# liuQuan98/APR

Measured on AMD Instinct MI355X. Metric: point-cloud pairs/sec (120k-pt KITTI frame, FCGF encode+match+SVD), higher is better.
Workload: dtype f32

## Files before the change

apr_amd/csrc/ransac.hip:

```cpp
#include <atomic>
#include <cstring>
#include <map>
#include <mutex>
#include <utility>

#include "common.h"
#include "irls.h"
#include "ransac_raw.h"

namespace {

__host__ __device__ inline uint64_t splitmix64(uint64_t z) {
  z = (z ^ (z >> 30)) * 0xBF58476D1CE4E5B9ull;
  z = (z ^ (z >> 27)) * 0x94D049BB133111EBull;
  return z ^ (z >> 31);
}

__host__ __device__ inline uint32_t sample_index(uint64_t seed, uint64_t it, int slot, uint32_t n) {
  uint64_t z = splitmix64(seed + (it * 4ull + (uint64_t)slot + 1ull) * 0x9E3779B97F4A7C15ull);
  return (uint32_t)(((z >> 32) * (uint64_t)n) >> 32);
}

__device__ inline void kabsch4(const double s[4][3], const double t[4][3], double T[12]) {
  double ms[3] = {0, 0, 0}, mt[3] = {0, 0, 0};
#pragma unroll
  for (int i = 0; i < 4; ++i)
#pragma unroll
    for (int d = 0; d < 3; ++d) {
      ms[d] += s[i][d];
      mt[d] += t[i][d];
    }
#pragma unroll
  for (int d = 0; d < 3; ++d) {
    ms[d] *= 0.25;
    mt[d] *= 0.25;
  }
  double S[3][3] = {{0, 0, 0}, {0, 0, 0}, {0, 0, 0}};
#pragma unroll
  for (int i = 0; i < 4; ++i)
#pragma unroll
    for (int a = 0; a < 3; ++a)
#pragma unroll
      for (int b = 0; b < 3; ++b) S[a][b] += (s[i][a] - ms[a]) * (t[i][b] - mt[b]);
  double A[4][4];
  A[0][0] = S[0][0] + S[1][1] + S[2][2];
  A[0][1] = S[1][2] - S[2][1];
  A[0][2] = S[2][0] - S[0][2];
  A[0][3] = S[0][1] - S[1][0];
  A[1][1] = S[0][0] - S[1][1] - S[2][2];
  A[1][2] = S[0][1] + S[1][0];
  A[1][3] = S[2][0] + S[0][2];
  A[2][2] = -S[0][0] + S[1][1] - S[2][2];
  A[2][3] = S[1][2] + S[2][1];
  A[3][3] = -S[0][0] - S[1][1] + S[2][2];
  A[1][0] = A[0][1]; A[2][0] = A[0][2]; A[3][0] = A[0][3];
  A[2][1] = A[1][2]; A[3][1] = A[1][3]; A[3][2] = A[2][3];
  double V[4][4] = {{1, 0, 0, 0}, {0, 1, 0, 0}, {0, 0, 1, 0}, {0, 0, 0, 1}};
  for (int sweep = 0; sweep < 12; ++sweep) {
    double off = 0.0;
#pragma unroll
    for (int p = 0; p < 4; ++p)
#pragma unroll
      for (int q2 = p + 1; q2 < 4; ++q2) off += A[p][q2] * A[p][q2];
    double diag = A[0][0] * A[0][0] + A[1][1] * A[1][1] + A[2][2] * A[2][2] + A[3][3] * A[3][3];
    if (off <= 1e-32 * diag || off == 0.0) break;
#pragma unroll
    for (int p = 0; p < 4; ++p)
#pragma unroll
      for (int q2 = p + 1; q2 < 4; ++q2) {
        double apq = A[p][q2];
        if (apq != 0.0) {
          double theta = (A[q2][q2] - A[p][p]) / (2.0 * apq);
          double tt = (theta >= 0.0 ? 1.0 : -1.0) / (fabs(theta) + sqrt(theta * theta + 1.0));
          double c = 1.0 / sqrt(tt * tt + 1.0), sn = tt * c;
#pragma unroll
          for (int k = 0; k < 4; ++k) {
            double akp = A[k][p], akq = A[k][q2];
            A[k][p] = c * akp - sn * akq;
            A[k][q2] = sn * akp + c * akq;
          }
#pragma unroll
          for (int k = 0; k < 4; ++k) {
            double apk = A[p][k], aqk = A[q2][k];
            A[p][k] = c * apk - sn * aqk;
            A[q2][k] = sn * apk + c * aqk;
          }
#pragma unroll
          for (int k = 0; k < 4; ++k) {
            double vkp = V[k][p], vkq = V[k][q2];
            V[k][p] = c * vkp - sn * vkq;
            V[k][q2] = sn * vkp + c * vkq;
          }
        }
      }
  }
  double best = A[0][0];
  double qw = V[0][0], qx = V[1][0], qy = V[2][0], qz = V[3][0];
#pragma unroll
  for (int j = 1; j < 4; ++j)
    if (A[j][j] > best) {
      best = A[j][j];
      qw = V[0][j]; qx = V[1][j]; qy = V[2][j]; qz = V[3][j];
    }
  double nq = 1.0 / sqrt(qw * qw + qx * qx + qy * qy + qz * qz);
  qw *= nq; qx *= nq; qy *= nq; qz *= nq;
  double R[3][3];
  R[0][0] = 1 - 2 * (qy * qy + qz * qz); R[0][1] = 2 * (qx * qy - qw * qz); R[0][2] = 2 * (qx * qz + qw * qy);
  R[1][0] = 2 * (qx * qy + qw * qz); R[1][1] = 1 - 2 * (qx * qx + qz * qz); R[1][2] = 2 * (qy * qz - qw * qx);
  R[2][0] = 2 * (qx * qz - qw * qy); R[2][1] = 2 * (qy * qz + qw * qx); R[2][2] = 1 - 2 * (qx * qx + qy * qy);
#pragma unroll
  for (int a = 0; a < 3; ++a) {
    T[a * 4 + 0] = R[a][0]; T[a * 4 + 1] = R[a][1]; T[a * 4 + 2] = R[a][2];
    T[a * 4 + 3] = mt[a] - (R[a][0] * ms[0] + R[a][1] * ms[1] + R[a][2] * ms[2]);
  }
}

constexpr int kMini = 32;
__host__ __device__ inline int64_t rec2_rows(int64_t n0) { return ((n0 + 1) / 2 + kMini - 1) / kMini * kMini; }

__global__ void k_pack_pairs(const float* __restrict__ xyz0, const float* __restrict__ xyz1, int64_t n1,
                             const long long* __restrict__ corr, int64_t n0, float4* __restrict__ rec,
                             float* __restrict__ rec2, unsigned* __restrict__ maxn2, float* __restrict__ rec2_live,
                             long long* __restrict__ corr_out) {
  int64_t i = (int64_t)blockIdx.x * blockDim.x + threadIdx.x;
  float sx = 0.f, sy = 0.f, sz = 0.f, tx = 3e18f, ty = 3e18f, tz = 3e18f, m = 0.f;
  if (i < n0) {
    long long j = corr[i];
    if (corr_out) {
      j &= 0xFFFFFFFFll;
      corr_out[i] = j;
    }
    if (j < 0 || j >= n1) j = 0;
    sx = xyz0[3 * i]; sy = xyz0[3 * i + 1]; sz = xyz0[3 * i + 2];
    tx = xyz1[3 * j]; ty = xyz1[3 * j + 1]; tz = xyz1[3 * j + 2];
    rec[2 * i] = make_float4(sx, sy, sz, 0.f);
    rec[2 * i + 1] = make_float4(tx, ty, tz, 0.f);
    m = fmaxf(sx * sx + sy * sy + sz * sz, tx * tx + ty * ty + tz * tz);
  }
  if (i < 2 * rec2_rows(n0)) {
    float* row = rec2 + (i >> 1) * 12 + (i & 1);
    row[0] = sx; row[2] = sy; row[4] = sz; row[6] = tx; row[8] = ty; row[10] = tz;
    float* lrow = rec2_live + (i >> 1) * 12 + (i & 1);
    lrow[0] = 0.f; lrow[2] = 0.f; lrow[4] = 0.f; lrow[6] = 3e18f; lrow[8] = 3e18f; lrow[10] = 3e18f;
  }
  for (int d = 32; d >= 1; d >>= 1) m = fmaxf(m, __shfl_xor(m, d));
  if ((threadIdx.x & 63) == 0 && m > 0.f) atomicMax(maxn2, __float_as_uint(m));
}

__device__ inline void load_samples(const float4* __restrict__ rec, uint64_t seed, long long it, uint32_t n0,
                                    double s[4][3], double t[4][3]) {
#pragma unroll
  for (int j = 0; j < 4; ++j) {
    const uint32_t i = sample_index(seed, (uint64_t)it, j, n0);
    const float4 a = rec[2 * (int64_t)i], b = rec[2 * (int64_t)i + 1];
    s[j][0] = (double)a.x; s[j][1] = (double)a.y; s[j][2] = (double)a.z;
    t[j][0] = (double)b.x; t[j][1] = (double)b.y; t[j][2] = (double)b.z;
  }
}

__device__ inline bool edge_reject(double a2, double b2, double r, double r2) {
  const double rb = b2 * r2;
  if (a2 < rb * (1.0 - 1e-12)) return true;
  if (a2 > rb * (1.0 + 1e-12)) return false;
  return sqrt(a2) < sqrt(b2) * r;
}

constexpr int kCandLists = 64;

__device__ inline bool sample_passes(const float4* __restrict__ rec, uint32_t n0, double edge_ratio, long long it,
                                     uint64_t seed) {
  float4 sf[4], tf[4];
  const double r2 = edge_ratio * edge_ratio;
  const float r2f = (float)r2;
  auto fetch = [&](int j) {
    const uint32_t i = sample_index(seed, (uint64_t)it, j, n0);
    sf[j] = rec[2 * (int64_t)i];
    tf[j] = rec[2 * (int64_t)i + 1];
  };
  auto edge_ok = [&](int a, int b) {
    const float dsx = sf[a].x - sf[b].x, dsy = sf[a].y - sf[b].y, dsz = sf[a].z - sf[b].z;
    const float dtx = tf[a].x - tf[b].x, dty = tf[a].y - tf[b].y, dtz = tf[a].z - tf[b].z;
    const float A = dsx * dsx + dsy * dsy + dsz * dsz, B = dtx * dtx + dty * dty + dtz * dtz;
    constexpr float lo = 1.f - 4e-6f, hi = 1.f + 4e-6f;
    const bool sound = (A == 0.f || A >= 1e-30f) && (B == 0.f || B >= 1e-30f) && A < 3e37f && B < 3e37f;
    if (sound && (A < r2f * B * lo || B < r2f * A * lo)) return false;
    if (sound && A > r2f * B * hi && B > r2f * A * hi) return true;
    const double ds2 = ((double)sf[a].x - (double)sf[b].x) * ((double)sf[a].x - (double)sf[b].x) +
                       ((double)sf[a].y - (double)sf[b].y) * ((double)sf[a].y - (double)sf[b].y) +
                       ((double)sf[a].z - (double)sf[b].z) * ((double)sf[a].z - (double)sf[b].z);
    const double dt2 = ((double)tf[a].x - (double)tf[b].x) * ((double)tf[a].x - (double)tf[b].x) +
                       ((double)tf[a].y - (double)tf[b].y) * ((double)tf[a].y - (double)tf[b].y) +
                       ((double)tf[a].z - (double)tf[b].z) * ((double)tf[a].z - (double)tf[b].z);
    return !(edge_reject(ds2, dt2, edge_ratio, r2) || edge_reject(dt2, ds2, edge_ratio, r2));
  };
  fetch(0);
  fetch(1);
  if (!edge_ok(0, 1)) return false;
  fetch(2);
  if (!(edge_ok(0, 2) && edge_ok(1, 2))) return false;
  fetch(3);
  return edge_ok(0, 3) && edge_ok(1, 3) && edge_ok(2, 3);
}

__device__ inline void append_candidate(bool ok, long long it, long long* __restrict__ cand, int* __restrict__ n_cand,
                                        int sub_cap) {
  const unsigned long long m = __ballot(ok);
  if (m) {
    const int lane = threadIdx.x & 63;
    const int list = blockIdx.x & (kCandLists - 1);
    int base = 0;
    if (lane == __ffsll((long long)m) - 1) base = atomicAdd(n_cand + list, __popcll(m));
    base = __shfl(base, __ffsll((long long)m) - 1);
    if (ok) cand[(int64_t)list * sub_cap + base + __popcll(m & ((1ull << lane) - 1ull))] = it;
  }
}

__global__ __launch_bounds__(256) void k_sample_check(const float4* __restrict__ rec, uint32_t n0, double edge_ratio,
                                                      long long it0, long long it1, uint64_t seed,
                                                      long long* __restrict__ cand, int* __restrict__ n_cand,
                                                      int sub_cap) {
  const long long it = it0 + (long long)blockIdx.x * blockDim.x + threadIdx.x;
  const bool ok = it < it1 && sample_passes(rec, n0, edge_ratio, it, seed);
  append_candidate(ok, it, cand, n_cand, sub_cap);
}

constexpr int kScreenThreads = 1024;
constexpr int kScreenPer = 2;
constexpr int kScreenRound = kScreenThreads * kScreenPer;
constexpr int kScreenQueue = 2 * kScreenRound;
constexpr int kScreenBits = 10;
constexpr int64_t kScreenMaxN0 = (160 * 1024 - kScreenQueue * 4 - 512) / 8;

__global__ void k_pack_small(const float4* __restrict__ rec, int64_t n0, const unsigned* __restrict__ maxn2,
                             unsigned long long* __restrict__ rec8) {
  const int64_t i = (int64_t)blockIdx.x * blockDim.x + threadIdx.x;
  if (i >= ((n0 + 31) & ~(int64_t)31)) return;
  if (i >= n0) {
    rec8[i] = 0ull;
    return;
  }
  const float R = sqrtf(__uint_as_float(*maxn2)) * 1.000001f;
  const float inv_h = R > 0.f ? (float)((1 << kScreenBits) - 1) / (2.f * R) : 0.f;
  auto q = [&](float c) {
    int u = (int)floorf((c + R) * inv_h);
    u = u < 0 ? 0 : (u > (1 << kScreenBits) - 1 ? (1 << kScreenBits) - 1 : u);
    return (unsigned)u;
  };
  const float4 a = rec[2 * i], b = rec[2 * i + 1];
  const unsigned lo = q(a.x) | (q(a.y) << kScreenBits) | (q(a.z) << (2 * kScreenBits));
  const unsigned hi = q(b.x) | (q(b.y) << kScreenBits) | (q(b.z) << (2 * kScreenBits));
  rec8[i] = (unsigned long long)lo | ((unsigned long long)hi << 32);
}

__device__ inline float cell_dist(unsigned a, unsigned b) {
  constexpr unsigned M = (1u << kScreenBits) - 1u;
  const int dx = (int)(a & M) - (int)(b & M), dy = (int)((a >> kScreenBits) & M) - (int)((b >> kScreenBits) & M),
            dz = (int)((a >> (2 * kScreenBits)) & M) - (int)((b >> (2 * kScreenBits)) & M);
  return __builtin_sqrtf((float)(dx * dx + dy * dy + dz * dz));
}

__device__ inline uint32_t sample_index_from(uint64_t z, uint32_t n) {
  z = (z ^ (z >> 30)) * 0xBF58476D1CE4E5B9ull;
  z = (z ^ (z >> 27)) * 0x94D049BB133111EBull;
  z ^= z >> 31;
  return (uint32_t)(((z >> 32) * (uint64_t)n) >> 32);
}

__global__ __launch_bounds__(kScreenThreads) void k_sample_screen(const float4* __restrict__ rec,
                                                                  const unsigned long long* __restrict__ rec8, uint32_t n0,
                                                                  double edge_ratio, long long it0, long long it1,
                                                                  long long per_wg, uint64_t seed,
                                                                  long long* __restrict__ cand, int* __restrict__ n_cand,
                                                                  int sub_cap) {
  extern __shared__ unsigned long long s_rec[];
  const uint32_t n0p = (n0 + 31u) & ~31u;
  unsigned* const s_q = reinterpret_cast<unsigned*>(s_rec + n0p);
  int& s_nq = *reinterpret_cast<int*>(s_q + kScreenQueue);
  const int tid = threadIdx.x, lane = tid & 63;
  {
    typedef unsigned long long u64x2 __attribute__((ext_vector_type(2)));
    const u64x2* src = reinterpret_cast<const u64x2*>(rec8);
    u64x2* dst = reinterpret_cast<u64x2*>(s_rec);
    const uint32_t nv = n0p >> 1;
    for (uint32_t i0 = tid; i0 < nv; i0 += 8 * kScreenThreads) {
      u64x2 t[8];
#pragma unroll
      for (int u = 0; u < 8; ++u)
        if (i0 + u * kScreenThreads < nv) t[u] = src[i0 + u * kScreenThreads];
#pragma unroll
      for (int u = 0; u < 8; ++u)
        if (i0 + u * kScreenThreads < nv) dst[i0 + u * kScreenThreads] = t[u];
    }
  }
  if (tid == 0) s_nq = 0;
  const long long base = it0 + (long long)blockIdx.x * per_wg;
  const long long end = (base + per_wg < it1) ? base + per_wg : it1;
  const float r = (float)edge_ratio, E = 1.75f;
  constexpr uint64_t G = 0x9E3779B97F4A7C15ull;
  auto drain = [&]() {
    const int nq = s_nq;
    for (int c0 = 0; c0 < nq; c0 += kScreenThreads) {
      const int c = c0 + tid;
      const long long it = c < nq ? base + (long long)s_q[c] : 0;
      const bool ok = c < nq && sample_passes(rec, n0, edge_ratio, it, seed);
      append_candidate(ok, it, cand, n_cand, sub_cap);
    }
  };
  __syncthreads();
  uint64_t z0 = seed + (uint64_t)(4 * (base + tid) + 1) * G;
  for (long long rb = base; rb < end; rb += kScreenRound) {
#pragma unroll
    for (int u = 0; u < kScreenPer; ++u) {
      const long long it = rb + u * kScreenThreads + tid;
      bool pass = false;
      if (it < end) {
        const unsigned long long a = s_rec[sample_index_from(z0, n0)];
        const unsigned long long b = s_rec[sample_index_from(z0 + G, n0)];
        const float Ds = cell_dist((unsigned)a, (unsigned)b), Dt = cell_dist((unsigned)(a >> 32), (unsigned)(b >> 32));
        pass = !(Ds + E < r * (Dt - E)) && !(Dt + E < r * (Ds - E));
      }
      z0 += (uint64_t)(4 * kScreenThreads) * G;
      const unsigned long long m = __ballot(pass);
      if (m) {
        int qb = 0;
        if (lane == __ffsll((long long)m) - 1) qb = atomicAdd(&s_nq, __popcll(m));
        qb = __shfl(qb, __ffsll((long long)m) - 1);
        if (pass) s_q[qb + __popcll(m & ((1ull << lane) - 1ull))] = (unsigned)(it - base);
      }
    }
    __syncthreads();
    const int nq_now = s_nq;
    __syncthreads();
    if (nq_now > kScreenQueue - kScreenRound) {
      drain();
      __syncthreads();
      if (tid == 0) s_nq = 0;
      __syncthreads();
    }
  }
  drain();
}

__global__ __launch_bounds__(256) void k_fit_check(const float4* __restrict__ rec, uint32_t n0, double thr_gt,
                                                   uint64_t seed, const long long* __restrict__ cand,
                                                   const int* __restrict__ n_cand, int sub_cap,
                                                   Hyp* __restrict__ hyps, int* __restrict__ n_valid, int cap) {
  __shared__ int s_off[kCandLists + 1];
  if (threadIdx.x < 64) {
    const int c = n_cand[threadIdx.x];
    const int incl = apr_wave_incl_scan(c);
    s_off[threadIdx.x + 1] = incl;
    if (threadIdx.x == 0) s_off[0] = 0;
  }
  __syncthreads();
  const int nc = s_off[kCandLists];
  for (int c = blockIdx.x * blockDim.x + threadIdx.x; c < nc; c += gridDim.x * blockDim.x) {
    int list = 0;
#pragma unroll
    for (int step = kCandLists / 2; step >= 1; step >>= 1)
      if (s_off[list + step] <= c) list += step;
    const long long it = cand[(int64_t)list * sub_cap + (c - s_off[list])];
    double s[4][3], t[4][3];
    load_samples(rec, seed, it, n0, s, t);
    double T[12];
    kabsch4(s, t, T);
    bool ok = true;
#pragma unroll
    for (int j = 0; j < 4; ++j) {
      double dx = T[0] * s[j][0] + T[1] * s[j][1] + T[2] * s[j][2] + T[3] - t[j][0];
      double dy = T[4] * s[j][0] + T[5] * s[j][1] + T[6] * s[j][2] + T[7] - t[j][1];
      double dz = T[8] * s[j][0] + T[9] * s[j][1] + T[10] * s[j][2] + T[11] - t[j][2];
      if (dx * dx + dy * dy + dz * dz > thr_gt) ok = false;
    }
    if (!ok) continue;
    const int slot = atomicAdd(n_valid, 1);
    if (slot < cap) {
#pragma unroll
      for (int k = 0; k < 12; ++k) hyps[slot].T[k] = T[k];
      hyps[slot].it = it;
      hyps[slot].inliers = 0;
      hyps[slot].err2 = 0.0;
    }
  }
}

constexpr int kGeoGrid = 2048;
struct GeoPart {
  double e2;
  int cnt;
  int pad;
};

__device__ inline int geo_parts(int nv, int64_t n0) {
  const int nchunk = (int)((n0 + 255) >> 8);
  int S = nv > 0 ? kGeoGrid / nv : 1;
  if (S > nchunk) S = nchunk;
  return S < 1 ? 1 : S;
}

constexpr int kScoreThreads = 256;
__device__ inline int score_parts(int nv, int64_t n0) {
  const int nblk = (int)((n0 + 4 * kScoreThreads - 1) / (4 * kScoreThreads));
  int S = nv > 0 ? kGeoGrid / nv : 1;
  if (S > nblk) S = nblk;
  return S < 1 ? 1 : S;
}

__global__ __launch_bounds__(kScoreThreads) void k_score(const float4* __restrict__ rec, int64_t n0, double thr_lt,
                                               Hyp* __restrict__ hyps, const int* __restrict__ sel_hdr,
                                               const int* __restrict__ sel, GeoPart* __restrict__ part) {
  constexpr int NW = kScoreThreads / 64;
  __shared__ int s_cnt[NW];
  __shared__ double s_e2[NW];
  const int lane = threadIdx.x & 63, wave = threadIdx.x >> 6;
  const int nv = sel_hdr[0];
  const int S = score_parts(nv, n0);
  const int64_t nblk = (n0 + 4 * kScoreThreads - 1) / (4 * kScoreThreads);
  for (int64_t item = blockIdx.x; item < (int64_t)nv * S; item += gridDim.x) {
    const int hs = (int)(item / S), pp = (int)(item - (int64_t)hs * S);
    const int h = sel[hs];
    const int64_t i_begin = (nblk * pp / S) * (4 * kScoreThreads);
    const int64_t i_end = min((long long)((nblk * (pp + 1) / S) * (4 * kScoreThreads)), (long long)n0);
    double T[12];
#pragma unroll
    for (int k = 0; k < 12; ++k) T[k] = hyps[h].T[k];
    int cnt = 0;
    double e2 = 0.0;
    for (int64_t i0 = i_begin + threadIdx.x; i0 < i_end; i0 += 4 * kScoreThreads) {
      float4 a[4], b[4];
#pragma unroll
      for (int u = 0; u < 4; ++u) {
        const int64_t i = i0 + u * kScoreThreads;
        if (i < i_end) {
          a[u] = rec[2 * i];
          b[u] = rec[2 * i + 1];
        }
      }
#pragma unroll
      for (int u = 0; u < 4; ++u) {
        if (i0 + u * kScoreThreads >= i_end) break;
        const double sx = a[u].x, sy = a[u].y, sz = a[u].z;
        double dx = T[0] * sx + T[1] * sy + T[2] * sz + T[3] - (double)b[u].x;
        double dy = T[4] * sx + T[5] * sy + T[6] * sz + T[7] - (double)b[u].y;
        double dz = T[8] * sx + T[9] * sy + T[10] * sz + T[11] - (double)b[u].z;
        double d2 = dx * dx + dy * dy + dz * dz;
        if (d2 < thr_lt) {
          ++cnt;
          e2 += d2;
        }
      }
    }
    for (int d = 32; d >= 1; d >>= 1) {
      cnt += __shfl_xor(cnt, d);
      e2 += __shfl_xor(e2, d);
    }
    if (lane == 0) {
      s_cnt[wave] = cnt;
      s_e2[wave] = e2;
    }
    __syncthreads();
    if (threadIdx.x == 0) {
      int c = 0;
      double e = 0.0;
      for (int w = 0; w < NW; ++w) {
        c += s_cnt[w];
        e += s_e2[w];
      }
      if (S == 1) {
        hyps[h].inliers = c;
        hyps[h].err2 = e;
      } else {
        part[item].cnt = c;
        part[item].e2 = e;
      }
    }
    __syncthreads();
  }
}

__global__ void k_score_finish(Hyp* __restrict__ hyps, const int* __restrict__ sel_hdr, const int* __restrict__ sel,
                               int64_t n0, const GeoPart* __restrict__ part) {
  const int nv = sel_hdr[0];
  const int S = score_parts(nv, n0);
  const int hs = blockIdx.x * blockDim.x + threadIdx.x;
  if (S == 1 || hs >= nv) return;
  int c = 0;
  double e = 0.0;
  for (int p = 0; p < S; ++p) {
    c += part[(int64_t)hs * S + p].cnt;
    e += part[(int64_t)hs * S + p].e2;
  }
  const int h = sel[hs];
  hyps[h].inliers = c;
  hyps[h].err2 = e;
}

typedef float f32x2 __attribute__((ext_vector_type(2)));

enum { kLiveCount = 0, kLiveMini = 1, kLiveWords = 2, kLiveNear = 3, kLiveFar = 4, kLiveInts = 8 };
constexpr double kPruneReach = 10.0;

__device__ inline void live_part(int blk, int nblk, const float4* __restrict__ rec, int64_t n0, double m_up,
                                 const Hyp* __restrict__ hyps, float4* __restrict__ rec_live, float* __restrict__ rec2_live,
                                 int* __restrict__ live) {
  const int lane = threadIdx.x & 63;
  const Hyp* hp = hyps;
  const double T0 = hp->T[0], T1 = hp->T[1], T2 = hp->T[2], T3 = hp->T[3], T4 = hp->T[4], T5 = hp->T[5];
  const double T6 = hp->T[6], T7 = hp->T[7], T8 = hp->T[8], T9 = hp->T[9], T10 = hp->T[10], T11 = hp->T[11];
  const double reach = m_up + kPruneReach, reach2 = reach * reach;
  const int64_t nround = (n0 + 255) & ~(int64_t)255;
  for (int64_t i = (int64_t)blk * blockDim.x + threadIdx.x; i < nround; i += (int64_t)nblk * blockDim.x) {
    bool keep = false;
    float4 a = make_float4(0.f, 0.f, 0.f, 0.f), b = a;
    if (i < n0) {
      a = rec[2 * i];
      b = rec[2 * i + 1];
      const double sx = a.x, sy = a.y, sz = a.z;
      const double dx = T0 * sx + T1 * sy + T2 * sz + T3 - (double)b.x;
      const double dy = T4 * sx + T5 * sy + T6 * sz + T7 - (double)b.y;
      const double dz = T8 * sx + T9 * sy + T10 * sz + T11 - (double)b.z;
      keep = !(dx * dx + dy * dy + dz * dz >= reach2);
    }
    const unsigned long long mk = __ballot(keep);
    int base = 0;
    if (lane == 0 && mk) base = atomicAdd(live + kLiveCount, __popcll(mk));
    base = __shfl(base, 0);
    if (keep) {
      const int pos = base + __popcll(mk & ((1ull << lane) - 1ull));
      rec_live[2 * (int64_t)pos] = a;
      rec_live[2 * (int64_t)pos + 1] = b;
      float* row = rec2_live + (int64_t)(pos >> 1) * 12 + (pos & 1);
      row[0] = a.x; row[2] = a.y; row[4] = a.z; row[6] = b.x; row[8] = b.y; row[10] = b.z;
    }
  }
}

__device__ inline void near_part(int blk, int nblk, const Hyp* __restrict__ hyps, int nv, const unsigned* __restrict__ maxn2,
                                 int prune, int* __restrict__ order_near, int* __restrict__ order_far,
                                 unsigned char* __restrict__ near_flag, int* __restrict__ live, unsigned* __restrict__ band,
                                 int nwords) {
  const int lane = threadIdx.x & 63;
  const double Mn = sqrt((double)__uint_as_float(*maxn2)) * (1.0 + 1e-6);
  const Hyp* r = hyps;
  const int nround = (nv + 255) & ~255;
  for (int h = blk * blockDim.x + threadIdx.x; h < nround; h += nblk * blockDim.x) {
    bool nr = false;
    if (h < nv && prune) {
      const Hyp* p = hyps + h;
      double f2 = 0.0, t2 = 0.0;
#pragma unroll
      for (int a = 0; a < 3; ++a) {
#pragma unroll
        for (int b = 0; b < 3; ++b) {
          const double d = p->T[4 * a + b] - r->T[4 * a + b];
          f2 += d * d;
        }
        const double dt = p->T[4 * a + 3] - r->T[4 * a + 3];
        t2 += dt * dt;
      }
      const double delta = (sqrt(f2) * Mn + sqrt(t2)) * (1.0 + 1e-9) + 1e-6;
      nr = delta <= kPruneReach;
    }
    const bool fr = h < nv && !nr;
    if (h < nv) {
      near_flag[h] = nr ? 1 : 0;
      for (int w = 0; w < nwords; ++w) band[(int64_t)h * nwords + w] = 0u;
    }
    const unsigned long long mn = __ballot(nr), mf = __ballot(fr);
    int bn = 0, bf = 0;
    if (lane == 0) {
      if (mn) bn = atomicAdd(live + kLiveNear, __popcll(mn));
      if (mf) bf = atomicAdd(live + kLiveFar, __popcll(mf));
    }
    bn = __shfl(bn, 0);
    bf = __shfl(bf, 0);
    if (nr) order_near[bn + __popcll(mn & ((1ull << lane) - 1ull))] = h;
    if (fr) order_far[bf + __popcll(mf & ((1ull << lane) - 1ull))] = h;
  }
}

__global__ __launch_bounds__(256) void k_prune(const float4* __restrict__ rec, int64_t n0, double m_up, Hyp* __restrict__ hyps,
                                               const int* __restrict__ n_valid, int cap, int few,
                                               const unsigned* __restrict__ maxn2, int prune, int n_live_blocks,
                                               float4* __restrict__ rec_live, float* __restrict__ rec2_live,
                                               int* __restrict__ live, int* __restrict__ order_near,
                                               int* __restrict__ order_far, unsigned char* __restrict__ near_flag,
                                               unsigned* __restrict__ band, int nwords) {
  const int nv = min(*n_valid, cap);
  if (nv <= few) return;
  if ((int)blockIdx.x < n_live_blocks)
    live_part((int)blockIdx.x, n_live_blocks, rec, n0, m_up, hyps, rec_live, rec2_live, live);
  else
    near_part((int)blockIdx.x - n_live_blocks, (int)gridDim.x - n_live_blocks, hyps, nv, maxn2, prune, order_near, order_far,
              near_flag, live, band, nwords);
}

__device__ inline int count_parts(int nblk, int nunits) {
  int S = (4096 + nblk - 1) / nblk;
  if (S > nunits) S = nunits;
  return S < 1 ? 1 : S;
}

__global__ __launch_bounds__(256) void k_count(const float* __restrict__ rec2_full, const float* __restrict__ rec2_live,
                                               int nwords, int nmini_full, double thr_lt,
                                               const unsigned* __restrict__ maxn2, Hyp* __restrict__ hyps,
                                               const int* __restrict__ n_valid, int cap, unsigned* __restrict__ band,
                                               int few, const int* __restrict__ order_near,
                                               const int* __restrict__ order_far, const int* __restrict__ live) {
  const int nv_all = min(*n_valid, cap);
  if (nv_all <= few) return;
  const int nvN = live[kLiveNear], nvF = live[kLiveFar], nminiN = (int)(rec2_rows(live[kLiveCount]) / kMini);
  const int nblkN = (nvN + 255) >> 8, nblkF = (nvF + 255) >> 8;
  const int SN = count_parts(nblkN > 0 ? nblkN : 1, nminiN > 0 ? nminiN : 1);
  const int SF = count_parts(nblkF > 0 ? nblkF : 1, nmini_full > 0 ? nmini_full : 1);
  const int itemsN = nminiN > 0 ? nblkN * SN : 0, itemsF = nblkF * SF;
  const int nwords_full = nwords;
  const float Mn = sqrtf(__uint_as_float(*maxn2)) * 1.000001f;
  const float thr = (float)thr_lt;
  for (int item0 = blockIdx.x; item0 < itemsN + itemsF; item0 += gridDim.x) {
    const bool isN = item0 < itemsN;
    const int item = isN ? item0 : item0 - itemsN;
    const int S = isN ? SN : SF, nv = isN ? nvN : nvF, nmini = isN ? nminiN : nmini_full;
    const int* __restrict__ order = isN ? order_near : order_far;
    const float* __restrict__ rec2 = isN ? rec2_live : rec2_full;
    const int hb = item / S, part = item - hb * S;
    const int m_begin = (int)((int64_t)nmini * part / S), m_stop = (int)((int64_t)nmini * (part + 1) / S);
    const int w_begin = m_begin >> 5, w_end = (m_stop + 31) >> 5;
    const int slot = hb * 256 + threadIdx.x;
    const bool act = slot < nv;
    const int h = order[act ? slot : nv - 1];
    const Hyp* hp = hyps + h;
    float T[12];
#pragma unroll
    for (int k = 0; k < 12; ++k) T[k] = (float)hp->T[k];
    const float tn = fmaxf(fabsf(T[3]), fmaxf(fabsf(T[7]), fabsf(T[11]))) * 1.000001f;
    const float e1 = 8.f * 5.9604645e-8f * (2.f * Mn + tn);
    const float b = (2.f * sqrtf(3.f * thr) * e1 + 3.f * e1 * e1 + 4.f * 5.9604645e-8f * thr) * 1.01f + 1e-30f;
    const float lo = thr - b, hi = thr + b;
    const f32x2 t0 = {T[0], T[0]}, t1 = {T[1], T[1]}, t2 = {T[2], T[2]}, t3 = {T[3], T[3]};
    const f32x2 t4 = {T[4], T[4]}, t5 = {T[5], T[5]}, t6 = {T[6], T[6]}, t7 = {T[7], T[7]};
    const f32x2 t8 = {T[8], T[8]}, t9 = {T[9], T[9]}, t10 = {T[10], T[10]}, t11 = {T[11], T[11]};
    int total = 0;
    for (int w = w_begin; w < w_end; ++w) {
// ... 1020 lines not shown
```

Before: 2793.

## Add staged cell-grid screening of third and fourth sample edges before full check

```diff
diff --git a/apr_amd/csrc/ransac.hip b/apr_amd/csrc/ransac.hip
--- a/apr_amd/csrc/ransac.hip
+++ b/apr_amd/csrc/ransac.hip
@@ -259,6 +259,12 @@
   return __builtin_sqrtf((float)(dx * dx + dy * dy + dz * dz));
 }
 
+__device__ inline bool cell_edge_rejected(unsigned long long a, unsigned long long b, float r) {
+  constexpr float E = 1.75f;
+  const float Ds = cell_dist((unsigned)a, (unsigned)b), Dt = cell_dist((unsigned)(a >> 32), (unsigned)(b >> 32));
+  return (Ds + E < r * (Dt - E)) || (Dt + E < r * (Ds - E));
+}
+
 __device__ inline uint32_t sample_index_from(uint64_t z, uint32_t n) {
   z = (z ^ (z >> 30)) * 0xBF58476D1CE4E5B9ull;
   z = (z ^ (z >> 27)) * 0x94D049BB133111EBull;
@@ -295,10 +301,44 @@
   if (tid == 0) s_nq = 0;
   const long long base = it0 + (long long)blockIdx.x * per_wg;
   const long long end = (base + per_wg < it1) ? base + per_wg : it1;
-  const float r = (float)edge_ratio, E = 1.75f;
+  const float r = (float)edge_ratio;
   constexpr uint64_t G = 0x9E3779B97F4A7C15ull;
-  auto drain = [&]() {
-    const int nq = s_nq;
+  auto enqueue = [&](bool pass, unsigned e) {
+    const unsigned long long m = __ballot(pass);
+    if (m) {
+      int qb = 0;
+      if (lane == __ffsll((long long)m) - 1) qb = atomicAdd(&s_nq, __popcll(m));
+      qb = __shfl(qb, __ffsll((long long)m) - 1);
+      if (pass) s_q[qb + __popcll(m & ((1ull << lane) - 1ull))] = e;
+    }
+  };
+  auto sift = [&](int n2, int nq, auto keep) {
+    if (tid == 0) s_nq = n2;
+    for (int c0 = n2; c0 < nq; c0 += kScreenThreads) {
+      const int c = c0 + tid;
+      const unsigned e = c < nq ? s_q[c] : 0u;
+      __syncthreads();
+      enqueue(c < nq && keep(seed + (uint64_t)(4 * (base + (long long)e) + 1) * G), e);
+    }
+    __syncthreads();
+    const int n = s_nq;
+    __syncthreads();
+    return n;
+  };
+  auto screen_rest = [&](int n2, int nq) {
+    nq = sift(n2, nq, [&](uint64_t z) {
+      const unsigned long long q2 = s_rec[sample_index_from(z + 2 * G, n0)];
+      return !cell_edge_rejected(s_rec[sample_index_from(z, n0)], q2, r) &&
+             !cell_edge_rejected(s_rec[sample_index_from(z + G, n0)], q2, r);
+    });
+    return sift(n2, nq, [&](uint64_t z) {
+      const unsigned long long q3 = s_rec[sample_index_from(z + 3 * G, n0)];
+      return !cell_edge_rejected(s_rec[sample_index_from(z, n0)], q3, r) &&
+             !cell_edge_rejected(s_rec[sample_index_from(z + G, n0)], q3, r) &&
+             !cell_edge_rejected(s_rec[sample_index_from(z + 2 * G, n0)], q3, r);
+    });
+  };
+  auto drain = [&](int nq) {
     for (int c0 = 0; c0 < nq; c0 += kScreenThreads) {
       const int c = c0 + tid;
       const long long it = c < nq ? base + (long long)s_q[c] : 0;
@@ -308,37 +348,32 @@
   };
   __syncthreads();
   uint64_t z0 = seed + (uint64_t)(4 * (base + tid) + 1) * G;
+  int nq = 0, n2 = 0;
   for (long long rb = base; rb < end; rb += kScreenRound) {
 #pragma unroll
     for (int u = 0; u < kScreenPer; ++u) {
       const long long it = rb + u * kScreenThreads + tid;
       bool pass = false;
-      if (it < end) {
-        const unsigned long long a = s_rec[sample_index_from(z0, n0)];
-        const unsigned long long b = s_rec[sample_index_from(z0 + G, n0)];
-        const float Ds = cell_dist((unsigned)a, (unsigned)b), Dt = cell_dist((unsigned)(a >> 32), (unsigned)(b >> 32));
-        pass = !(Ds + E < r * (Dt - E)) && !(Dt + E < r * (Ds - E));
+      if (it < end)
+        pass = !cell_edge_rejected(s_rec[sample_index_from(z0, n0)], s_rec[sample_index_from(z0 + G, n0)], r);
+      z0 += (uint64_t)(4 * kScreenThreads) * G;
+      enqueue(pass, (unsigned)(it - base));
+    }
+    __syncthreads();
+    nq = s_nq;
+    __syncthreads();
+    if (nq > kScreenQueue - kScreenRound) {
+      nq = n2 = screen_rest(n2, nq);
+      if (nq > kScreenQueue - kScreenRound) {
+        drain(nq);
+        __syncthreads();
+        if (tid == 0) s_nq = 0;
+        __syncthreads();
+        nq = n2 = 0;
       }
-      z0 += (uint64_t)(4 * kScreenThreads) * G;
-      const unsigned long long m = __ballot(pass);
-      if (m) {
-        int qb = 0;
-        if (lane == __ffsll((long long)m) - 1) qb = atomicAdd(&s_nq, __popcll(m));
-        qb = __shfl(qb, __ffsll((long long)m) - 1);
-        if (pass) s_q[qb + __popcll(m & ((1ull << lane) - 1ull))] = (unsigned)(it - base);
-      }
-    }
-    __syncthreads();
-    const int nq_now = s_nq;
-    __syncthreads();
-    if (nq_now > kScreenQueue - kScreenRound) {
-      drain();
-      __syncthreads();
-      if (tid == 0) s_nq = 0;
-      __syncthreads();
-    }
-  }
-  drain();
+    }
+  }
+  drain(screen_rest(n2, nq));
 }
 
 __global__ __launch_bounds__(256) void k_fit_check(const float4* __restrict__ rec, uint32_t n0, double thr_gt,
```

Result: slower. 2408 (-13.8%).
